# egyptdj/graph-neural-mapping

Hardware: AMD Instinct MI355X
Metric: graphs/sec fwd+bwd, 400-node dense FC graphs, hidden_dim 64, 5 layers (higher is better)
Workload: dtype f32

## Files before the change

graph-neural-mapping_amd/csrc/linear.hip:

```cpp
#include "gnm_split.h"

static bool lin_force_generic() { static const bool v = getenv("GNM_LIN_GENERIC") != nullptr; return v; }
static bool lin_no_stream() { static const bool v = getenv("GNM_LIN_NO_STREAM") != nullptr; return v; }

struct LinArgs {
    const float* X;
    const float* W;
    const float* bias;
    float* Z;
    const float* pro_scale;
    const float* pro_shift;
    double* stats_partial;
    int ldx, ldw, ldz;
    int N, K, H;
    int w_kmajor;
    int pro_relu;
    unsigned long long* stamps;
    int stat_rows;
    int stage_out;
    const float* mZ; const float* m_scale; const float* m_shift; const float* m_mean; const float* m_rstd;
    int ldmz;
};

__host__ __device__ __forceinline__ int lin_first_tile_of(int wave, int groups, int rows, int nwg, int b) {
// ... 1980 lines not shown
                        }
                        dacc[c][r] = g;
                    }
            }
#pragma unroll
            for (int c = 0; c < KT; ++c)
#pragma unroll
                for (int r = 0; r < 16; ++r) Xs[((r & 3) + 8 * (r >> 2) + 4 * h) * XS + 32 * c + i] = dacc[c][r];
            __builtin_amdgcn_fence(__ATOMIC_RELEASE, "wavefront");
            __builtin_amdgcn_wave_barrier();
            __builtin_amdgcn_fence(__ATOMIC_ACQUIRE, "wavefront");
            if constexpr (STATS && !SAMEZ) {
                __builtin_amdgcn_sched_barrier(0);
                const float4 lsc = *reinterpret_cast<const float4*>(p.s_scale + 4 * oc4);
                const float4 lsh = *reinterpret_cast<const float4*>(p.s_shift + 4 * oc4);
                const float4 lmu = *reinterpret_cast<const float4*>(p.s_mean + 4 * oc4);
                const float4 lrs = *reinterpret_cast<const float4*>(p.s_rstd + 4 * oc4);
                constexpr int NJ = 32 / OR, HB = NJ > 4 ? 4 : NJ;
#pragma unroll
                for (int j0 = 0; j0 < NJ; j0 += HB) {
                float4 zl[HB];
#pragma unroll
                for (int j = 0; j < HB; ++j) {
                    const int grow = min(r0 + orow0 + (j0 + j) * OR, nlast);
                    zl[j] = *reinterpret_cast<const float4*>(p.sZ + (size_t)grow * p.ldsz + 4 * oc4);
                }
#pragma unroll
                for (int j = 0; j < HB; ++j) {
                    const int row = orow0 + (j0 + j) * OR;
                    float4 g = *reinterpret_cast<const float4*>(Xs + row * XS + 4 * oc4);
                    const float4 z = zl[j];
                    if (z.x * lsc.x + lsh.x <= 0.f) g.x = 0.f;
                    if (z.y * lsc.y + lsh.y <= 0.f) g.y = 0.f;
                    if (z.z * lsc.z + lsh.z <= 0.f) g.z = 0.f;
                    if (z.w * lsc.w + lsh.w <= 0.f) g.w = 0.f;
                    if (r0 + row < p.N) {
                        *reinterpret_cast<float4*>(p.dA + (size_t)(r0 + row) * p.lda + 4 * oc4) = g;
                        ss1.x += g.x; ss1.y += g.y; ss1.z += g.z; ss1.w += g.w;
                        ss2.x += g.x * ((z.x - lmu.x) * lrs.x); ss2.y += g.y * ((z.y - lmu.y) * lrs.y);
                        ss2.z += g.z * ((z.z - lmu.z) * lrs.z); ss2.w += g.w * ((z.w - lmu.w) * lrs.w);
                    }
                }
                }
            } else if constexpr (NARROW) {
                for (int idx = lane; idx < 32 * p.K; idx += 64) {
                    const int row = idx / p.K, col = idx - row * p.K;
                    if (r0 + row < p.N) p.dA[(size_t)(r0 + row) * p.lda + col] = Xs[row * XS + col];
                }
            } else {
#pragma unroll
                for (int idx = lane; idx < 32 * O4; idx += 64) {
                    const int row = idx / O4, oc = idx - row * O4;
                    if (r0 + row < p.N)
                        *reinterpret_cast<float4*>(p.dA + (size_t)(r0 + row) * p.lda + 4 * oc) =
                            *reinterpret_cast<const float4*>(Xs + row * XS + 4 * oc);
                }
            }
            __builtin_amdgcn_fence(__ATOMIC_RELEASE, "wavefront");
            __builtin_amdgcn_wave_barrier();
        }
        GNM_LSTAMP(6 + 5 * min(tk, 11))
        ++tk;
    }
    GNM_LSTAMP(62)

    if constexpr (STATS) {
        __syncthreads();
        double* sred = reinterpret_cast<double*>(smem);
        if constexpr (SAMEZ) {
#pragma unroll
            for (int c = 0; c < KT; ++c) {
                double d1 = (double)cs1[c], d2 = (double)cs2[c];
                d1 += __shfl_xor(d1, 32, 64);
                d2 += __shfl_xor(d2, 32, 64);
                if (h == 0) {
                    sred[(wave * 2 + 0) * KP + 32 * c + i] = d1;
                    sred[(wave * 2 + 1) * KP + 32 * c + i] = d2;
                }
            }
        }
        float v1[4] = {ss1.x, ss1.y, ss1.z, ss1.w}, v2[4] = {ss2.x, ss2.y, ss2.z, ss2.w};
#pragma unroll
        for (int c = 0; c < (SAMEZ ? 0 : 4); ++c) {
            double d1 = (double)v1[c], d2 = (double)v2[c];
#pragma unroll
            for (int off = O4; off < 64; off <<= 1) {
                d1 += __shfl_xor(d1, off, 64);
                d2 += __shfl_xor(d2, off, 64);
            }
            if (lane < O4) {
                sred[(wave * 2 + 0) * KP + 4 * oc4 + c] = d1;
                sred[(wave * 2 + 1) * KP + 4 * oc4 + c] = d2;
            }
        }
        __syncthreads();
        for (int idx = tid; idx < 2 * KP; idx += 256) {
            const int which = idx / KP, col = idx - which * KP;
            double sum = 0.0;
            for (int w = 0; w < 4; ++w) sum += sred[(w * 2 + which) * KP + col];
            p.s_partial[((size_t)blockIdx.x * 2 + which) * p.K + col] = sum;
        }
    }

    lb_combine<HT, KT, 1, NARROW>(smem, wacc, dbacc, p.partial, p.H, p.K, 0, tid, lane, wave);
    GNM_LSTAMP(63)
}

template <int KT, int HT, bool SPLITD = false>
__global__ void __launch_bounds__(256, 2) gnm_linear_bwd_pipe_kernel(const LbArgs p) {
    static_assert(!SPLITD || (KT == 2 && HT == 2), "SPLITD: K = H = 64 only");
    using L = LbLds<KT, HT, SPLITD, true>;
    constexpr int KP = L::KP, HP = L::HP, XS = L::XS, EW = L::EW;
    constexpr int H4 = HP / 4;
    constexpr int NLD = (32 * H4) / 64;
    constexpr int RSTEP = 64 / H4;
    constexpr int KH = HP / 2;
    constexpr int O4 = KP / 4;
    extern __shared__ __attribute__((aligned(16))) char smem[];
    float* Wt = reinterpret_cast<float*>(smem);
    gnm_u32x4* Wp = reinterpret_cast<gnm_u32x4*>(smem);
    float* Xs_all = reinterpret_cast<float*>(smem + L::xs_off);
    float* coef = reinterpret_cast<float*>(smem + L::coef_off);
    const int tid = threadIdx.x;
    const int lane = tid & 63;
    const int wave = __builtin_amdgcn_readfirstlane(tid >> 6);
    const int i = lane & 31, h = lane >> 5;
    float* Xs = Xs_all + wave * 32 * XS;
    if constexpr (SPLITD) {
        lin_stage_planes<KT, 32, true, false>(Wp, EW, p.W, p.ldw, 0, tid, 256);
    } else {
        for (int idx = tid; idx < HP * KP; idx += 256) {
            const int hh = idx / KP, k = idx - hh * KP;
            Wt[idx] = p.W[(size_t)hh * p.ldw + k];
        }
    }
    lb_stage_coef<HP, false>(coef, p.mean, p.rstd, p.cA, p.m1, p.m2, nullptr, tid, 256);
    const int c4 = lane % H4, lrow0 = lane / H4;
    float psc[KT], psh[KT];
#pragma unroll
    for (int b = 0; b < KT; ++b) {
        psc[b] = p.pro_scale ? p.pro_scale[32 * b + i] : 1.f;
        psh[b] = p.pro_scale ? p.pro_shift[32 * b + i] : 0.f;
    }
    __builtin_amdgcn_s_waitcnt(0x0F70);
    __syncthreads();
    f32x16 wacc[HT][KT];
#pragma unroll
    for (int a = 0; a < HT; ++a)
#pragma unroll
        for (int b = 0; b < KT; ++b)
#pragma unroll
            for (int r = 0; r < 16; ++r) wacc[a][b][r] = 0.f;
    float dbacc[HT];
#pragma unroll
    for (int a = 0; a < HT; ++a) dbacc[a] = 0.f;

    const int ntiles = (p.N + 31) / 32;
    const int tstride = gridDim.x * 4;
    const int gz_voff_g = (lrow0 * p.ldg + 4 * c4) * 4, gz_step_g = RSTEP * p.ldg * 4;
    const int gz_voff_z = (lrow0 * p.ldz + 4 * c4) * 4, gz_step_z = RSTEP * p.ldz * 4;
    const int x_voff = (h * p.ldx + i) * 4;
    const int out_voff = ((lane / O4) * p.lda + 4 * (lane % O4)) * 4, out_step = (64 / O4) * p.lda * 4;
    const float* dxbase = p.dA ? p.dA : p.G;

    gnm_u32x4 g4[NLD], z4[NLD];
    auto load_gz = [&](int tile) {
        const long long row0 = (long long)tile * 32;
        const long long rows = min((long long)p.N - row0, 32LL);
        const __amdgpu_buffer_rsrc_t rg = gnm_tile_rsrc(p.G + row0 * p.ldg, rows, p.ldg, HP);
        const __amdgpu_buffer_rsrc_t rz = gnm_tile_rsrc(p.Z + row0 * p.ldz, rows, p.ldz, HP);
#pragma unroll
        for (int j = 0; j < NLD; ++j) {
            g4[j] = __builtin_amdgcn_raw_buffer_load_b128(rg, gz_voff_g, j * gz_step_g, 0);
            z4[j] = __builtin_amdgcn_raw_buffer_load_b128(rz, gz_voff_z, j * gz_step_z, 0);
        }
    };
    auto do_tile = [&](int t, int t_next) {
        const int r0 = t * 32;
        const int rows = min(p.N - r0, 32);
        const float4 mu = *reinterpret_cast<const float4*>(coef + 4 * c4);
        const float4 rs = *reinterpret_cast<const float4*>(coef + HP + 4 * c4);
        const float4 ca = *reinterpret_cast<const float4*>(coef + 2 * HP + 4 * c4);
        const float4 a1 = *reinterpret_cast<const float4*>(coef + 3 * HP + 4 * c4);
        const float4 a2 = *reinterpret_cast<const float4*>(coef + 4 * HP + 4 * c4);
#pragma unroll
        for (int j = 0; j < NLD; ++j) {
            const int lrow = lrow0 + j * RSTEP;
            const float4 gj = __builtin_bit_cast(float4, g4[j]), zj = __builtin_bit_cast(float4, z4[j]);
            float4 d;
            d.x = ca.x * (gj.x - a1.x - (zj.x - mu.x) * rs.x * a2.x);
            d.y = ca.y * (gj.y - a1.y - (zj.y - mu.y) * rs.y * a2.y);
            d.z = ca.z * (gj.z - a1.z - (zj.z - mu.z) * rs.z * a2.z);
            d.w = ca.w * (gj.w - a1.w - (zj.w - mu.w) * rs.w * a2.w);
            if (lrow >= rows) d = make_float4(0.f, 0.f, 0.f, 0.f);
            *reinterpret_cast<float4*>(Xs + lrow * XS + 4 * c4) = d;
        }
        __builtin_amdgcn_fence(__ATOMIC_RELEASE, "wavefront");
        __builtin_amdgcn_wave_barrier();
        __builtin_amdgcn_fence(__ATOMIC_ACQUIRE, "wavefront");
        float xv[16][KT];
        {
            const __amdgpu_buffer_rsrc_t rx = gnm_tile_rsrc(p.X + (size_t)r0 * p.ldx, rows, p.ldx, KP);
#pragma unroll
            for (int s = 0; s < 16; ++s)
#pragma unroll
                for (int b = 0; b < KT; ++b)
                    xv[s][b] = __uint_as_float(__builtin_amdgcn_raw_buffer_load_b32(rx, x_voff, (2 * s * p.ldx + 32 * b) * 4, 0));
        }
        __builtin_amdgcn_sched_barrier(0);
        f32x16 dacc[KT];
        if constexpr (SPLITD) {
#pragma unroll
            for (int c = 0; c < KT; ++c)
#pragma unroll
                for (int r = 0; r < 16; ++r) dacc[c][r] = 0.f;
            lin_dgrad_split<KT, HP>(dacc, Xs, XS, Wp, i, h, lane);
        } else {
            float a[KH];
#pragma unroll
            for (int j = 0; j < KH / 4; ++j) {
                const float4 v = *reinterpret_cast<const float4*>(Xs + i * XS + KH * h + 4 * j);
                a[4 * j + 0] = v.x; a[4 * j + 1] = v.y; a[4 * j + 2] = v.z; a[4 * j + 3] = v.w;
            }
#pragma unroll
            for (int c = 0; c < KT; ++c)
#pragma unroll
                for (int r = 0; r < 16; ++r) dacc[c][r] = 0.f;
            const float* wrow = Wt + (size_t)(KH * h) * KP + i;
#pragma unroll
            for (int s = 0; s < KH; ++s) {
#pragma unroll
                for (int c = 0; c < KT; ++c)
                    dacc[c] = __builtin_amdgcn_mfma_f32_32x32x2f32(a[s], wrow[s * KP + 32 * c], dacc[c], 0, 0, 0);
            }
        }
        load_gz(t_next);
#pragma unroll
        for (int s = 0; s < 16; ++s) {
            float av[HT];
            const int krow = 2 * s + h;
#pragma unroll
            for (int a = 0; a < HT; ++a) av[a] = Xs[krow * XS + 32 * a + i];
            float xf[KT];
#pragma unroll
            for (int b = 0; b < KT; ++b) {
                float x = xv[s][b];
                if (p.pro_scale) {
                    x = x * psc[b] + psh[b];
                    if (p.pro_relu) x = gnm_relu(x);
                }
                xf[b] = x;
            }
#pragma unroll
            for (int a = 0; a < HT; ++a) {
                dbacc[a] += av[a];
#pragma unroll
                for (int b = 0; b < KT; ++b)
                    wacc[a][b] = __builtin_amdgcn_mfma_f32_32x32x2f32(av[a], xf[b], wacc[a][b], 0, 0, 0);
            }
        }
        __builtin_amdgcn_fence(__ATOMIC_RELEASE, "wavefront");
        __builtin_amdgcn_wave_barrier();
#pragma unroll
        for (int c = 0; c < KT; ++c)
#pragma unroll
            for (int r = 0; r < 16; ++r) Xs[((r & 3) + 8 * (r >> 2) + 4 * h) * XS + 32 * c + i] = dacc[c][r];
        __builtin_amdgcn_fence(__ATOMIC_RELEASE, "wavefront");
        __builtin_amdgcn_wave_barrier();
        __builtin_amdgcn_fence(__ATOMIC_ACQUIRE, "wavefront");
        {
            const __amdgpu_buffer_rsrc_t rd = gnm_tile_rsrc(dxbase + (p.dA ? (size_t)r0 * p.lda : 0), p.dA ? rows : 0, p.lda, KP);
#pragma unroll
            for (int st = 0; st < (32 * O4) / 64; ++st) {
                const int idx = lane + 64 * st;
                const int row = idx / O4, oc = idx - row * O4;
                const gnm_u32x4 v = *reinterpret_cast<const gnm_u32x4*>(Xs + row * XS + 4 * oc);
                __builtin_amdgcn_raw_buffer_store_b128(v, rd, out_voff + st * out_step, 0, 0);
            }
        }
        __builtin_amdgcn_fence(__ATOMIC_RELEASE, "wavefront");
        __builtin_amdgcn_wave_barrier();
    };
    {
        int t = lin_first_tile(wave, 1, gridDim.x);
        load_gz(t);
        if (t < ntiles) {
            do_tile(t, t + tstride);
            for (t += tstride; t < ntiles; t += tstride) do_tile(t, t + tstride);
        }
    }

    lb_combine<HT, KT, 1, false>(smem, wacc, dbacc, p.partial, p.H, p.K, 0, tid, lane, wave);
}

template <int KT, int HT, bool SPLITD = false>
static int launch_lb_pipe(const LbArgs& a, int grid, hipStream_t s) {
    const size_t lds = LbLds<KT, HT, SPLITD, true>::total;
    GNM_ALLOW_FULL_LDS((&gnm_linear_bwd_pipe_kernel<KT, HT, SPLITD>));
    hipLaunchKernelGGL((gnm_linear_bwd_pipe_kernel<KT, HT, SPLITD>), dim3(grid), dim3(256), lds, s, a);
    GNM_CHECK_LAUNCH();
    return GNM_OK;
}

struct LbSzLds {
    using L = LbLds<2, 2, true, true>;
    static constexpr size_t half_off = L::body;
    static constexpr size_t body = L::body + (size_t)4 * 16 * L::XS * 4;
    static constexpr size_t total = body > lb_dump_bytes(2, 2, 4) ? body : lb_dump_bytes(2, 2, 4);
    static_assert(total <= 80 * 1024, "two workgroups share a CU");
};
__global__ void __launch_bounds__(256, 2) gnm_linear_bwd_pipe_sz_kernel(const LbArgs p) {
    constexpr int KT = 2, HT = 2;
    using L = LbLds<KT, HT, true, true>;
    constexpr int KP = L::KP, HP = L::HP, XS = L::XS, EW = L::EW;
    constexpr int H4 = HP / 4;
    constexpr int NLD = (32 * H4) / 64;
    constexpr int RSTEP = 64 / H4;
    constexpr int O4 = KP / 4;
    extern __shared__ __attribute__((aligned(16))) char smem[];
    gnm_u32x4* Wp = reinterpret_cast<gnm_u32x4*>(smem);
    float* Xs_all = reinterpret_cast<float*>(smem + L::xs_off);
    float* coef = reinterpret_cast<float*>(smem + L::coef_off);
    const int tid = threadIdx.x;
    const int lane = tid & 63;
    const int wave = __builtin_amdgcn_readfirstlane(tid >> 6);
    const int i = lane & 31, h = lane >> 5;
    float* Xs = Xs_all + wave * 32 * XS;
    float* Hs = reinterpret_cast<float*>(smem + LbSzLds::half_off) + wave * 16 * XS;
    lin_stage_planes<KT, 32, true, false>(Wp, EW, p.W, p.ldw, 0, tid, 256);
    lb_stage_coef<HP, false>(coef, p.mean, p.rstd, p.cA, p.m1, p.m2, nullptr, tid, 256);
    const int c4 = lane % H4, lrow0 = lane / H4;
    float psc[KT], psh[KT], cmu[KT], crs[KT], cs1[KT], cs2[KT];
#pragma unroll
    for (int b = 0; b < KT; ++b) {
        psc[b] = p.pro_scale ? p.pro_scale[32 * b + i] : 1.f;
        psh[b] = p.pro_scale ? p.pro_shift[32 * b + i] : 0.f;
        cmu[b] = p.s_mean[32 * b + i];
        crs[b] = p.s_rstd[32 * b + i];
        cs1[b] = 0.f; cs2[b] = 0.f;
    }
    __builtin_amdgcn_s_waitcnt(0x0F70);
    __syncthreads();
    f32x16 wacc[HT][KT];
#pragma unroll
    for (int a = 0; a < HT; ++a)
#pragma unroll
        for (int b = 0; b < KT; ++b)
#pragma unroll
            for (int r = 0; r < 16; ++r) wacc[a][b][r] = 0.f;
    float dbacc[HT];
#pragma unroll
    for (int a = 0; a < HT; ++a) dbacc[a] = 0.f;

    const int ntiles = (p.N + 31) / 32;
    const int tstride = gridDim.x * 4;
    const int gz_voff_g = (lrow0 * p.ldg + 4 * c4) * 4, gz_step_g = RSTEP * p.ldg * 4;
    const int gz_voff_z = (lrow0 * p.ldz + 4 * c4) * 4, gz_step_z = RSTEP * p.ldz * 4;
    const int x_voff = (4 * h * p.ldx + i) * 4;
    const int out_voff = ((lane / O4) * p.lda + 4 * (lane % O4)) * 4;

    gnm_u32x4 g4[NLD], z4[NLD];
    auto load_gz = [&](int tile) {
        const long long row0 = (long long)tile * 32;
        const long long rows = min((long long)p.N - row0, 32LL);
        const __amdgpu_buffer_rsrc_t rg = gnm_tile_rsrc(p.G + row0 * p.ldg, rows, p.ldg, HP);
        const __amdgpu_buffer_rsrc_t rz = gnm_tile_rsrc(p.Z + row0 * p.ldz, rows, p.ldz, HP);
#pragma unroll
        for (int j = 0; j < NLD; ++j) {
            g4[j] = __builtin_amdgcn_raw_buffer_load_b128(rg, gz_voff_g, j * gz_step_g, 0);
            z4[j] = __builtin_amdgcn_raw_buffer_load_b128(rz, gz_voff_z, j * gz_step_z, 0);
        }
    };
    auto do_tile = [&](int t, int t_next) {
        const int r0 = t * 32;
        const int rows = min(p.N - r0, 32);
        const float4 mu = *reinterpret_cast<const float4*>(coef + 4 * c4);
        const float4 rs = *reinterpret_cast<const float4*>(coef + HP + 4 * c4);
        const float4 ca = *reinterpret_cast<const float4*>(coef + 2 * HP + 4 * c4);
        const float4 a1 = *reinterpret_cast<const float4*>(coef + 3 * HP + 4 * c4);
        const float4 a2 = *reinterpret_cast<const float4*>(coef + 4 * HP + 4 * c4);
#pragma unroll
        for (int j = 0; j < NLD; ++j) {
            const int lrow = lrow0 + j * RSTEP;
            const float4 gj = __builtin_bit_cast(float4, g4[j]), zj = __builtin_bit_cast(float4, z4[j]);
            float4 d;
            d.x = ca.x * (gj.x - a1.x - (zj.x - mu.x) * rs.x * a2.x);
            d.y = ca.y * (gj.y - a1.y - (zj.y - mu.y) * rs.y * a2.y);
            d.z = ca.z * (gj.z - a1.z - (zj.z - mu.z) * rs.z * a2.z);
            d.w = ca.w * (gj.w - a1.w - (zj.w - mu.w) * rs.w * a2.w);
            if (lrow >= rows) d = make_float4(0.f, 0.f, 0.f, 0.f);
            *reinterpret_cast<float4*>(Xs + lrow * XS + 4 * c4) = d;
        }
        __builtin_amdgcn_fence(__ATOMIC_RELEASE, "wavefront");
        __builtin_amdgcn_wave_barrier();
        __builtin_amdgcn_fence(__ATOMIC_ACQUIRE, "wavefront");
        float xv[16][KT];
        {
            const __amdgpu_buffer_rsrc_t rx = gnm_tile_rsrc(p.X + (size_t)r0 * p.ldx, rows, p.ldx, KP);
#pragma unroll
            for (int s = 0; s < 16; ++s)
#pragma unroll
                for (int b = 0; b < KT; ++b)
                    xv[s][b] = __uint_as_float(__builtin_amdgcn_raw_buffer_load_b32(
                        rx, x_voff, (((s & 3) + 8 * (s >> 2)) * p.ldx + 32 * b) * 4, 0));
        }
        __builtin_amdgcn_sched_barrier(0);
        f32x16 dacc[KT];
#pragma unroll
        for (int c = 0; c < KT; ++c)
#pragma unroll
            for (int r = 0; r < 16; ++r) dacc[c][r] = 0.f;
        lin_dgrad_split<KT, HP>(dacc, Xs, XS, Wp, i, h, lane);
        {
            const __amdgpu_buffer_rsrc_t rd = gnm_tile_rsrc(p.dA + (size_t)r0 * p.lda, rows, p.lda, KP);
            auto mask_sum = [&](int c, int r) {
                const float z = xv[r][c];
                float g = dacc[c][r];
                if (z * psc[c] + psh[c] <= 0.f) g = 0.f;
                if ((r & 3) + 8 * (r >> 2) + 4 * h < rows) {
                    cs1[c] += g;
                    cs2[c] += g * ((z - cmu[c]) * crs[c]);
                }
                return g;
            };
#pragma unroll
            for (int q = 0; q < 2; ++q) {
                float gq[KT][8];
#pragma unroll
                for (int c = 0; c < KT; ++c)
#pragma unroll
                    for (int r = 0; r < 8; ++r) gq[c][r] = mask_sum(c, 8 * q + r);
#pragma unroll
                for (int c = 0; c < KT; ++c)
#pragma unroll
                    for (int r = 0; r < 8; ++r) Hs[((r & 3) + 8 * (r >> 2) + 4 * h) * XS + 32 * c + i] = gq[c][r];
                __builtin_amdgcn_fence(__ATOMIC_RELEASE, "wavefront");
                __builtin_amdgcn_wave_barrier();
                __builtin_amdgcn_fence(__ATOMIC_ACQUIRE, "wavefront");
#pragma unroll
                for (int st = 0; st < (16 * O4) / 64; ++st) {
                    const int idx = lane + 64 * st;
                    const int row = idx / O4, oc = idx - row * O4;
                    const gnm_u32x4 v = *reinterpret_cast<const gnm_u32x4*>(Hs + row * XS + 4 * oc);
                    __builtin_amdgcn_raw_buffer_store_b128(v, rd, out_voff + (16 * q + (64 / O4) * st) * p.lda * 4, 0, 0);
                }
                __builtin_amdgcn_fence(__ATOMIC_RELEASE, "wavefront");
                __builtin_amdgcn_wave_barrier();
            }
        }
        __builtin_amdgcn_sched_barrier(0);
        load_gz(t_next);
        __builtin_amdgcn_sched_barrier(0);
#pragma unroll
        for (int s = 0; s < 16; ++s) {
            float av[HT];
            const int krow = (s & 3) + 8 * (s >> 2) + 4 * h;
#pragma unroll
            for (int a = 0; a < HT; ++a) av[a] = Xs[krow * XS + 32 * a + i];
            float xf[KT];
#pragma unroll
            for (int b = 0; b < KT; ++b) {
                float x = xv[s][b];
                if (p.pro_scale) {
                    x = x * psc[b] + psh[b];
                    if (p.pro_relu) x = gnm_relu(x);
                }
                xf[b] = x;
            }
#pragma unroll
            for (int a = 0; a < HT; ++a) {
                dbacc[a] += av[a];
#pragma unroll
                for (int b = 0; b < KT; ++b)
                    wacc[a][b] = __builtin_amdgcn_mfma_f32_32x32x2f32(av[a], xf[b], wacc[a][b], 0, 0, 0);
            }
        }
        __builtin_amdgcn_fence(__ATOMIC_RELEASE, "wavefront");
        __builtin_amdgcn_wave_barrier();
    };
    {
        int t = lin_first_tile(wave, 1, gridDim.x);
        load_gz(t);
        if (t < ntiles) {
            do_tile(t, t + tstride);
            for (t += tstride; t < ntiles; t += tstride) do_tile(t, t + tstride);
        }
    }

    __syncthreads();
    double* sred = reinterpret_cast<double*>(smem);
#pragma unroll
    for (int c = 0; c < KT; ++c) {
        double d1 = (double)cs1[c], d2 = (double)cs2[c];
        d1 += __shfl_xor(d1, 32, 64);
        d2 += __shfl_xor(d2, 32, 64);
        if (h == 0) {
            sred[(wave * 2 + 0) * KP + 32 * c + i] = d1;
            sred[(wave * 2 + 1) * KP + 32 * c + i] = d2;
        }
    }
    __syncthreads();
    for (int idx = tid; idx < 2 * KP; idx += 256) {
        const int which = idx / KP, col = idx - which * KP;
        double sum = 0.0;
        for (int w = 0; w < 4; ++w) sum += sred[(w * 2 + which) * KP + col];
        p.s_partial[((size_t)blockIdx.x * 2 + which) * p.K + col] = sum;
    }

    lb_combine<HT, KT, 1, false>(smem, wacc, dbacc, p.partial, p.H, p.K, 0, tid, lane, wave);
}

static int launch_lb_pipe_sz(const LbArgs& a, int grid, hipStream_t s) {
    const size_t lds = LbSzLds::total;
    GNM_ALLOW_FULL_LDS((&gnm_linear_bwd_pipe_sz_kernel));
    hipLaunchKernelGGL(gnm_linear_bwd_pipe_sz_kernel, dim3(grid), dim3(256), lds, s, a);
    GNM_CHECK_LAUNCH();
    return GNM_OK;
}

template <int KT, int HT, bool STATS, bool NARROW = false, bool SAMEZ = false, bool SPLITD = false>
static int launch_lb(const LbArgs& a, int grid, hipStream_t s) {
    const size_t lds = LbLds<KT, HT, SPLITD, false>::total;
    GNM_ALLOW_FULL_LDS((&gnm_linear_bwd_fused_kernel<KT, HT, STATS, NARROW, SAMEZ, SPLITD>));
    hipLaunchKernelGGL((gnm_linear_bwd_fused_kernel<KT, HT, STATS, NARROW, SAMEZ, SPLITD>), dim3(grid), dim3(256), lds, s, a);
    GNM_CHECK_LAUNCH();
    return GNM_OK;
}

__device__ __forceinline__ void rz_load_g(float (&g)[2][16], const float* G, int ldg, int N, int tile, int g_voff) {
    const long long row0 = (long long)tile * 32;
    const long long rows = min((long long)N - row0, 32LL);
    const __amdgpu_buffer_rsrc_t rg = gnm_tile_rsrc(G + row0 * ldg, rows, ldg, 64);
#pragma unroll
    for (int r = 0; r < 16; ++r)
#pragma unroll
        for (int a = 0; a < 2; ++a)
            g[a][r] = __uint_as_float(__builtin_amdgcn_raw_buffer_load_b32(rg, g_voff + 128 * a, ((r & 3) + 8 * (r >> 2)) * ldg * 4, 0));
}
__device__ __forceinline__ float rz_bn_bwd(f32x16& dz, const float (&g)[16], const float* coef, int col, int rows, float* Xs,
                                           int xs, int h) {
    const float mu = coef[col], rs = coef[64 + col], ca = coef[128 + col], a1 = coef[192 + col], a2 = coef[256 + col],
                bz = coef[320 + col];
    float dsum = 0.f;
#pragma unroll
    for (int r = 0; r < 16; ++r) {
        const int lrow = (r & 3) + 8 * (r >> 2) + 4 * h;
        const float z = dz[r] + bz;
        float d = ca * (g[r] - a1 - (z - mu) * rs * a2);
        if (lrow >= rows) d = 0.f;
        dz[r] = d;
        dsum += d;
        Xs[lrow * xs + col] = d;
    }
    return dsum;
}

__global__ void __launch_bounds__(kRzWaves * 64) gnm_linear_bwd_rz_kernel(const LbArgs p) {
    using L = RzLds<false>;
    constexpr int KP = 64, HP = 64, XS = L::XS, EW = 512, NW = kRzWaves, NT = NW * 64;
    static_assert(L::EWF == EW && L::EWB == EW, "both plane images hold 4 m x 2 c x 64 entries");
    extern __shared__ __attribute__((aligned(16))) char smem[];
    gnm_u32x4* Wf = reinterpret_cast<gnm_u32x4*>(smem);
    gnm_u32x4* Wb = reinterpret_cast<gnm_u32x4*>(smem + L::wb_off);
    float* Xs_all = reinterpret_cast<float*>(smem + L::xs_off);
    float* coef = reinterpret_cast<float*>(smem + L::coef_off);
    float* psv = reinterpret_cast<float*>(smem + L::psv_off);
    const int tid = threadIdx.x;
    const int lane = tid & 63;
    const int wave = __builtin_amdgcn_readfirstlane(tid >> 6);
    const int i = lane & 31, h = lane >> 5;
    float* Xs = Xs_all + wave * 32 * XS;
    const bool pro = p.pro_scale != nullptr;
    GNM_RSTAMP(0)
    lin_stage_planes<2, 32, false, false>(Wf, EW, p.W, p.ldw, 0, tid, NT);
    lin_stage_planes<2, 32, true, false>(Wb, EW, p.W, p.ldw, 0, tid, NT);
    lb_stage_coef<64, true>(coef, p.mean, p.rstd, p.cA, p.m1, p.m2, p.bias, tid, NT);
    for (int idx = tid; idx < 64; idx += NT) {
        psv[idx] = pro ? p.pro_scale[idx] : 1.f;
        psv[64 + idx] = pro ? p.pro_shift[idx] : 0.f;
    }
    float psc[2], psh[2];
#pragma unroll
    for (int b = 0; b < 2; ++b) {
        psc[b] = pro ? p.pro_scale[32 * b + i] : 1.f;
        psh[b] = pro ? p.pro_shift[32 * b + i] : 0.f;
    }
    __builtin_amdgcn_s_waitcnt(0x0F70);
    __syncthreads();
    GNM_RSTAMP(1)
    int tk = 0;

    f32x16 wacc[2][2];
#pragma unroll
    for (int a = 0; a < 2; ++a)
#pragma unroll
        for (int b = 0; b < 2; ++b)
#pragma unroll
            for (int r = 0; r < 16; ++r) wacc[a][b][r] = 0.f;
    float dbacc[2] = {0.f, 0.f};

    const int gw = lin_first_tile(wave, NW / 4, p.part_rows);
    const int ntiles = (p.N + 31) / 32;
    const int tstride = p.part_rows * 4;
    const int g_voff = (4 * h * p.ldg + i) * 4;
    const int xa_voff = (i * p.ldx + 32 * h) * 4;
    const int xc_voff = (4 * h * p.ldx + i) * 4;
    const int out_voff = ((lane >> 4) * p.lda + 4 * (lane & 15)) * 4, out_step = 4 * p.lda * 4;

    float g[2][16];
    gnm_u32x4 xa[4][2];
    auto load_next_x = [&](int tile) {
        const long long row0 = (long long)tile * 32;
        const long long rows = min((long long)p.N - row0, 32LL);
        const __amdgpu_buffer_rsrc_t rx = gnm_tile_rsrc(p.X + row0 * p.ldx, rows, p.ldx, KP);
#pragma unroll
        for (int m = 0; m < 4; ++m) {
            xa[m][0] = __builtin_amdgcn_raw_buffer_load_b128(rx, xa_voff, 32 * m, 0);
            xa[m][1] = __builtin_amdgcn_raw_buffer_load_b128(rx, xa_voff, 32 * m + 16, 0);
        }
    };
    auto do_tile = [&](int t, int t_next) {
        const int r0 = t * 32;
        const int rows = min(p.N - r0, 32);
        GNM_RSTAMP(2 + 6 * min(tk, 9))
        f32x16 dz[2];
#pragma unroll
        for (int c = 0; c < 2; ++c)
#pragma unroll
            for (int r = 0; r < 16; ++r) dz[c][r] = 0.f;
#pragma unroll
        for (int m = 0; m < 4; ++m) {
            const float4 v0 = __builtin_bit_cast(float4, xa[m][0]), v1 = __builtin_bit_cast(float4, xa[m][1]);
            float f[8] = {v0.x, v0.y, v0.z, v0.w, v1.x, v1.y, v1.z, v1.w};
            if (pro) {
                const int k0 = 32 * h + 8 * m;
#pragma unroll
                for (int q = 0; q < 2; ++q) {
                    const float4 sc = *reinterpret_cast<const float4*>(psv + k0 + 4 * q);
                    const float4 sh = *reinterpret_cast<const float4*>(psv + 64 + k0 + 4 * q);
                    f[4 * q + 0] = f[4 * q + 0] * sc.x + sh.x; f[4 * q + 1] = f[4 * q + 1] * sc.y + sh.y;
                    f[4 * q + 2] = f[4 * q + 2] * sc.z + sh.z; f[4 * q + 3] = f[4 * q + 3] * sc.w + sh.w;
                }
                if (p.pro_relu) {
#pragma unroll
                    for (int j = 0; j < 8; ++j) f[j] = gnm_relu(f[j]);
                }
            }
            gnm_bf16x8 a1, a2, a3;
            gnm_split8(f, a1, a2, a3);
#pragma unroll
            for (int c = 0; c < 2; ++c) gnm_mma6_planes(dz[c], a1, a2, a3, Wf, EW, (m * 2 + c) * 64 + lane);
        }
        GNM_RSTAMP(3 + 6 * min(tk, 9))
#pragma unroll
        for (int a = 0; a < 2; ++a) dbacc[a] += rz_bn_bwd(dz[a], g[a], coef, 32 * a + i, rows, Xs, XS, h);
        __builtin_amdgcn_fence(__ATOMIC_RELEASE, "wavefront");
        __builtin_amdgcn_wave_barrier();
        __builtin_amdgcn_fence(__ATOMIC_ACQUIRE, "wavefront");
        float xv[16][2];
        {
            const __amdgpu_buffer_rsrc_t rx = gnm_tile_rsrc(p.X + (size_t)r0 * p.ldx, rows, p.ldx, KP);
#pragma unroll
            for (int r = 0; r < 16; ++r)
#pragma unroll
                for (int b = 0; b < 2; ++b)
                    xv[r][b] = __uint_as_float(__builtin_amdgcn_raw_buffer_load_b32(rx, xc_voff + 128 * b, ((r & 3) + 8 * (r >> 2)) * p.ldx * 4, 0));
        }
        __builtin_amdgcn_sched_barrier(0);
        GNM_RSTAMP(4 + 6 * min(tk, 9))
        f32x16 dacc[2];
#pragma unroll
        for (int c = 0; c < 2; ++c)
#pragma unroll
            for (int r = 0; r < 16; ++r) dacc[c][r] = 0.f;
        lin_dgrad_split<2, HP>(dacc, Xs, XS, Wb, i, h, lane);
        __builtin_amdgcn_fence(__ATOMIC_RELEASE, "wavefront");
        __builtin_amdgcn_wave_barrier();
        GNM_RSTAMP(5 + 6 * min(tk, 9))
#pragma unroll
        for (int c = 0; c < 2; ++c)
#pragma unroll
            for (int r = 0; r < 16; ++r) Xs[((r & 3) + 8 * (r >> 2) + 4 * h) * XS + 32 * c + i] = dacc[c][r];
        __builtin_amdgcn_fence(__ATOMIC_RELEASE, "wavefront");
        __builtin_amdgcn_wave_barrier();
        __builtin_amdgcn_fence(__ATOMIC_ACQUIRE, "wavefront");
        {
            const __amdgpu_buffer_rsrc_t rd = gnm_tile_rsrc(p.dA + (size_t)r0 * p.lda, rows, p.lda, KP);
#pragma unroll
            for (int st = 0; st < 8; ++st) {
                const int idx = lane + 64 * st;
                const int row = idx >> 4, oc = idx & 15;
                const gnm_u32x4 v = *reinterpret_cast<const gnm_u32x4*>(Xs + row * XS + 4 * oc);
                __builtin_amdgcn_raw_buffer_store_b128(v, rd, out_voff + st * out_step, 0, 0);
            }
        }
        __builtin_amdgcn_fence(__ATOMIC_RELEASE, "wavefront");
        __builtin_amdgcn_wave_barrier();
        GNM_RSTAMP(6 + 6 * min(tk, 9))
        rz_load_g(g, p.G, p.ldg, p.N, t_next, (int)g_voff);
        load_next_x(t_next);
#pragma unroll
        for (int m = 0; m < 2; ++m) {
            gnm_bf16x8 dp[2][3], xp[2][3];
#pragma unroll
            for (int a = 0; a < 2; ++a) {
                float f[8];
#pragma unroll
                for (int j = 0; j < 8; ++j) f[j] = dz[a][8 * m + j];
                gnm_split8(f, dp[a][0], dp[a][1], dp[a][2]);
#pragma unroll
                for (int j = 0; j < 8; ++j) {
                    float x = xv[8 * m + j][a];
                    if (pro) {
                        x = x * psc[a] + psh[a];
                        if (p.pro_relu) x = gnm_relu(x);
                    }
                    f[j] = x;
                }
                gnm_split8(f, xp[a][0], xp[a][1], xp[a][2]);
            }
#pragma unroll
            for (int a = 0; a < 2; ++a)
#pragma unroll
                for (int b = 0; b < 2; ++b) gnm_mma6(wacc[a][b], dp[a][0], dp[a][1], dp[a][2], xp[b][0], xp[b][1], xp[b][2]);
        }
        GNM_RSTAMP(7 + 6 * min(tk, 9))
        ++tk;
    };
    {
        int t = gw;
        load_next_x(t);
        rz_load_g(g, p.G, p.ldg, p.N, t, (int)g_voff);
        if (t < ntiles) {
            do_tile(t, t + tstride);
            for (t += tstride; t < ntiles; t += tstride) do_tile(t, t + tstride);
        }
    }
    __builtin_amdgcn_s_waitcnt(0x0F70);
    GNM_RSTAMP(62)

    lb_combine<2, 2, 2, false>(smem, wacc, dbacc, p.partial, HP, KP, p.part_rows, tid, lane, wave);
    GNM_RSTAMP(63)
}

static int launch_lb_rz(const LbArgs& a, int grid, hipStream_t s) {
    const size_t lds = RzLds<false>::total;
    GNM_ALLOW_FULL_LDS((&gnm_linear_bwd_rz_kernel));
    hipLaunchKernelGGL(gnm_linear_bwd_rz_kernel, dim3((grid + 1) / 2), dim3(kRzWaves * 64), lds, s, a);
    GNM_CHECK_LAUNCH();
    return GNM_OK;
}

__global__ void __launch_bounds__(kRzWaves * 64) gnm_linear_bwd_rzn_kernel(const LbArgs p) {
    using L = RzLds<true>;
    constexpr int HP = 64, XS = L::XS, NW = kRzWaves, NT = NW * 64, TILE = 16 * 64;
    extern __shared__ __attribute__((aligned(16))) char smem[];
    gnm_u32x4* Wf = reinterpret_cast<gnm_u32x4*>(smem);
    gnm_u32x4* Wb = reinterpret_cast<gnm_u32x4*>(smem + L::wb_off);
    float* Xs_all = reinterpret_cast<float*>(smem + L::xs_off);
    float* coef = reinterpret_cast<float*>(smem + L::coef_off);
    const int tid = threadIdx.x;
    const int lane = tid & 63;
    const int wave = __builtin_amdgcn_readfirstlane(tid >> 6);
    const int i = lane & 31, h = lane >> 5;
    float* Xs = Xs_all + wave * 32 * XS;
    const int K = p.K;
    lin_stage_planes<2, 8, false, true>(Wf, L::EWF, p.W, p.ldw, K, tid, NT);
    lin_stage_planes<1, 32, true, true>(Wb, L::EWB, p.W, p.ldw, K, tid, NT);
    lb_stage_coef<64, true>(coef, p.mean, p.rstd, p.cA, p.m1, p.m2, p.bias, tid, NT);
    __builtin_amdgcn_s_waitcnt(0x0F70);
    __syncthreads();

    f32x16 wacc[2];
#pragma unroll
    for (int a = 0; a < 2; ++a)
#pragma unroll
        for (int r = 0; r < 16; ++r) wacc[a][r] = 0.f;
    float dbacc[2] = {0.f, 0.f};
    const int gw = lin_first_tile(wave, NW / 4, p.part_rows);
    const int ntiles = (p.N + 31) / 32;
    const int tstride = p.part_rows * 4;
    const unsigned g_voff = (unsigned)((4 * h * p.ldg + i) * 4);
    const unsigned kclip = 0x80000000u;
    const unsigned xc_voff = i < K ? (unsigned)((4 * h * p.ldx + i) * 4) : kclip;
    const unsigned da_voff = i < K ? (unsigned)((4 * h * p.lda + i) * 4) : kclip;
// ... 288 lines not shown
```

Before: 424,600.

## Use bf16x3 split MFMA for weight-grad in fused backward kernel

Replaces the fp32 32x32x2 MFMA weight-gradient accumulation in the split-dgrad backward kernel with a three-way bf16 split (gnm_mma6) over 8-row chunks, giving higher MFMA throughput while keeping near-fp32 accuracy. It also moves the prologue scale/shift/ReLU into the masking pass and splits the next-tile G/Z prefetch into two halves interleaved with the MFMA loop. Lane-derived indices are recomputed inside the tile body via an opaque register to ease register pressure. The extra split arithmetic and the packing instructions could offset the MFMA gains.

```diff
diff --git a/graph-neural-mapping_amd/csrc/linear.hip b/graph-neural-mapping_amd/csrc/linear.hip
--- a/graph-neural-mapping_amd/csrc/linear.hip
+++ b/graph-neural-mapping_amd/csrc/linear.hip
@@ -2306,6 +2306,20 @@
     return GNM_OK;
 }
 
+__device__ __forceinline__ void lb_split8_pairs(const float (&f)[8], gnm_bf16x8& p1, gnm_bf16x8& p2, gnm_bf16x8& p3) {
+    gnm_u32x4 q1, q2, q3;
+#pragma unroll
+    for (int j = 0; j < 4; ++j) {
+        unsigned a1[2], a2[2], a3[2];
+        gnm_split3(f[2 * j], a1[0], a2[0], a3[0]);
+        gnm_split3(f[2 * j + 1], a1[1], a2[1], a3[1]);
+        q1[j] = gnm_bf16_pair(a1[0], a1[1]);
+        q2[j] = gnm_bf16_pair(a2[0], a2[1]);
+        q3[j] = gnm_bf16_pair(a3[0], a3[1]);
+        __builtin_amdgcn_sched_barrier(0);
+    }
+    p1 = __builtin_bit_cast(gnm_bf16x8, q1); p2 = __builtin_bit_cast(gnm_bf16x8, q2); p3 = __builtin_bit_cast(gnm_bf16x8, q3);
+}
 struct LbSzLds {
     using L = LbLds<2, 2, true, true>;
     static constexpr size_t half_off = L::body;
@@ -2343,6 +2357,7 @@
         crs[b] = p.s_rstd[32 * b + i];
         cs1[b] = 0.f; cs2[b] = 0.f;
     }
+    const bool pro_relu = p.pro_scale && p.pro_relu;
     __builtin_amdgcn_s_waitcnt(0x0F70);
     __syncthreads();
     f32x16 wacc[HT][KT];
@@ -2358,19 +2373,17 @@
 
     const int ntiles = (p.N + 31) / 32;
     const int tstride = gridDim.x * 4;
-    const int gz_voff_g = (lrow0 * p.ldg + 4 * c4) * 4, gz_step_g = RSTEP * p.ldg * 4;
-    const int gz_voff_z = (lrow0 * p.ldz + 4 * c4) * 4, gz_step_z = RSTEP * p.ldz * 4;
-    const int x_voff = (4 * h * p.ldx + i) * 4;
-    const int out_voff = ((lane / O4) * p.lda + 4 * (lane % O4)) * 4;
+    const int gz_step_g = RSTEP * p.ldg * 4, gz_step_z = RSTEP * p.ldz * 4;
 
     gnm_u32x4 g4[NLD], z4[NLD];
-    auto load_gz = [&](int tile) {
+    auto load_gz_half = [&](int tile, int half, int ln) {
+        const int gz_voff_g = ((ln / H4) * p.ldg + 4 * (ln % H4)) * 4, gz_voff_z = ((ln / H4) * p.ldz + 4 * (ln % H4)) * 4;
         const long long row0 = (long long)tile * 32;
         const long long rows = min((long long)p.N - row0, 32LL);
         const __amdgpu_buffer_rsrc_t rg = gnm_tile_rsrc(p.G + row0 * p.ldg, rows, p.ldg, HP);
         const __amdgpu_buffer_rsrc_t rz = gnm_tile_rsrc(p.Z + row0 * p.ldz, rows, p.ldz, HP);
 #pragma unroll
-        for (int j = 0; j < NLD; ++j) {
+        for (int j = (NLD / 2) * half; j < (NLD / 2) * (half + 1); ++j) {
             g4[j] = __builtin_amdgcn_raw_buffer_load_b128(rg, gz_voff_g, j * gz_step_g, 0);
             z4[j] = __builtin_amdgcn_raw_buffer_load_b128(rz, gz_voff_z, j * gz_step_z, 0);
         }
@@ -2378,6 +2391,11 @@
     auto do_tile = [&](int t, int t_next) {
         const int r0 = t * 32;
         const int rows = min(p.N - r0, 32);
+        int ln = lane;
+        asm volatile("" : "+v"(ln));
+        const int i = ln & 31, h = ln >> 5, c4 = ln % H4, lrow0 = ln / H4;
+        const int x_voff = (4 * h * p.ldx + i) * 4;
+        const int out_v = ((ln / O4) * p.lda + 4 * (ln % O4)) * 4;
         const float4 mu = *reinterpret_cast<const float4*>(coef + 4 * c4);
         const float4 rs = *reinterpret_cast<const float4*>(coef + HP + 4 * c4);
         const float4 ca = *reinterpret_cast<const float4*>(coef + 2 * HP + 4 * c4);
@@ -2392,7 +2410,7 @@
             d.y = ca.y * (gj.y - a1.y - (zj.y - mu.y) * rs.y * a2.y);
             d.z = ca.z * (gj.z - a1.z - (zj.z - mu.z) * rs.z * a2.z);
             d.w = ca.w * (gj.w - a1.w - (zj.w - mu.w) * rs.w * a2.w);
-            if (lrow >= rows) d = make_float4(0.f, 0.f, 0.f, 0.f);
+            if (lrow0 >= rows - j * RSTEP) d = make_float4(0.f, 0.f, 0.f, 0.f);
             *reinterpret_cast<float4*>(Xs + lrow * XS + 4 * c4) = d;
         }
         __builtin_amdgcn_fence(__ATOMIC_RELEASE, "wavefront");
@@ -2414,17 +2432,19 @@
         for (int c = 0; c < KT; ++c)
 #pragma unroll
             for (int r = 0; r < 16; ++r) dacc[c][r] = 0.f;
-        lin_dgrad_split<KT, HP>(dacc, Xs, XS, Wp, i, h, lane);
+        lin_dgrad_split<KT, HP>(dacc, Xs, XS, Wp, i, h, ln);
         {
             const __amdgpu_buffer_rsrc_t rd = gnm_tile_rsrc(p.dA + (size_t)r0 * p.lda, rows, p.lda, KP);
             auto mask_sum = [&](int c, int r) {
                 const float z = xv[r][c];
+                const float f = z * psc[c] + psh[c];
                 float g = dacc[c][r];
-                if (z * psc[c] + psh[c] <= 0.f) g = 0.f;
-                if ((r & 3) + 8 * (r >> 2) + 4 * h < rows) {
+                if (f <= 0.f) g = 0.f;
+                if (4 * h < rows - ((r & 3) + 8 * (r >> 2))) {
                     cs1[c] += g;
                     cs2[c] += g * ((z - cmu[c]) * crs[c]);
                 }
+                xv[r][c] = pro_relu ? gnm_relu(f) : f;
                 return g;
             };
 #pragma unroll
@@ -2443,40 +2463,48 @@
                 __builtin_amdgcn_fence(__ATOMIC_ACQUIRE, "wavefront");
 #pragma unroll
                 for (int st = 0; st < (16 * O4) / 64; ++st) {
-                    const int idx = lane + 64 * st;
+                    const int idx = ln + 64 * st;
                     const int row = idx / O4, oc = idx - row * O4;
                     const gnm_u32x4 v = *reinterpret_cast<const gnm_u32x4*>(Hs + row * XS + 4 * oc);
-                    __builtin_amdgcn_raw_buffer_store_b128(v, rd, out_voff + (16 * q + (64 / O4) * st) * p.lda * 4, 0, 0);
+                    __builtin_amdgcn_raw_buffer_store_b128(v, rd, out_v + (16 * q + (64 / O4) * st) * p.lda * 4, 0, 0);
                 }
                 __builtin_amdgcn_fence(__ATOMIC_RELEASE, "wavefront");
                 __builtin_amdgcn_wave_barrier();
             }
         }
         __builtin_amdgcn_sched_barrier(0);
-        load_gz(t_next);
+        load_gz_half(t_next, 0, ln);
         __builtin_amdgcn_sched_barrier(0);
 #pragma unroll
-        for (int s = 0; s < 16; ++s) {
-            float av[HT];
-            const int krow = (s & 3) + 8 * (s >> 2) + 4 * h;
-#pragma unroll
-            for (int a = 0; a < HT; ++a) av[a] = Xs[krow * XS + 32 * a + i];
-            float xf[KT];
+        for (int q = 0; q < 2; ++q) {
+            gnm_bf16x8 xp[KT][3];
 #pragma unroll
             for (int b = 0; b < KT; ++b) {
-                float x = xv[s][b];
-                if (p.pro_scale) {
-                    x = x * psc[b] + psh[b];
-                    if (p.pro_relu) x = gnm_relu(x);
-                }
-                xf[b] = x;
+                float f[8];
+#pragma unroll
+                for (int j = 0; j < 8; ++j) f[j] = xv[8 * q + j][b];
+                lb_split8_pairs(f, xp[b][0], xp[b][1], xp[b][2]);
+                __builtin_amdgcn_sched_barrier(0);
             }
 #pragma unroll
             for (int a = 0; a < HT; ++a) {
-                dbacc[a] += av[a];
-#pragma unroll
-                for (int b = 0; b < KT; ++b)
-                    wacc[a][b] = __builtin_amdgcn_mfma_f32_32x32x2f32(av[a], xf[b], wacc[a][b], 0, 0, 0);
+                float f[8];
+#pragma unroll
+                for (int j = 0; j < 8; ++j) {
+                    f[j] = Xs[(16 * q + (j & 3) + 8 * (j >> 2) + 4 * h) * XS + 32 * a + i];
+                    dbacc[a] += f[j];
+                }
+                gnm_bf16x8 dp[3];
+                lb_split8_pairs(f, dp[0], dp[1], dp[2]);
+                __builtin_amdgcn_sched_barrier(0);
+#pragma unroll
+                for (int b = 0; b < KT; ++b) gnm_mma6(wacc[a][b], dp[0], dp[1], dp[2], xp[b][0], xp[b][1], xp[b][2]);
+                __builtin_amdgcn_sched_barrier(0);
+            }
+            if (q == 0) {
+                __builtin_amdgcn_sched_barrier(0);
+                load_gz_half(t_next, 1, ln);
+                __builtin_amdgcn_sched_barrier(0);
             }
         }
         __builtin_amdgcn_fence(__ATOMIC_RELEASE, "wavefront");
@@ -2484,7 +2512,8 @@
     };
     {
         int t = lin_first_tile(wave, 1, gridDim.x);
-        load_gz(t);
+        load_gz_half(t, 0, lane);
+        load_gz_half(t, 1, lane);
         if (t < ntiles) {
             do_tile(t, t + tstride);
             for (t += tstride; t < ntiles; t += tstride) do_tile(t, t + tstride);
```

Measured after the change: 424,400 (median of 3 runs). About the same (-0.0%).
